# AVianEco/Softspoken

Measured on AMD Instinct MI355X. Metric: audio-seconds processed/sec (whole node), 16 kHz mono, higher is better.
Workload: dtype f16x2

## Files before the change

### softspoken_amd/csrc/conv1s.hip

```cpp
#include "kernels.h"
#include "stream16.h"
#include <algorithm>
#include <type_traits>

namespace ss {

static constexpr int kFPitch = 36;
static constexpr int kFPatch = (kMaxRows + 5) * kFPitch;

__device__ __forceinline__ float s1_from_left(float v) {
    return __builtin_bit_cast(float, __builtin_amdgcn_update_dpp(0, __builtin_bit_cast(int, v), 0x138, 0xf, 0xf, true));
}
__device__ __forceinline__ float s1_from_right(float v) {
    return __builtin_bit_cast(float, __builtin_amdgcn_update_dpp(0, __builtin_bit_cast(int, v), 0x130, 0xf, 0xf, true));
}

struct S1Row { u32x4 f[2][2]; };

template <bool TRACK>
__global__ __launch_bounds__(64 * kS1Waves) __attribute__((amdgpu_waves_per_eu(2, 2)))
void conv1_stream_kernel(ConvArgs a, int rows_per_unit, int total_units) {
    extern __shared__ __attribute__((aligned(16))) char smem[];
    char* sW = smem;
    char* sK = smem + 2 * kBank;
    char* sPrev = sK + 3 * 1024;
    float* sF = (float*)(sPrev + kS1Waves * 4096);

    const int tid = threadIdx.x, lane = tid & 63, wave = __builtin_amdgcn_readfirstlane(tid >> 6);
    const int hh = lane >> 5, m = lane & 31;
    for (int p = tid; p < 2 * kBank / 16; p += 64 * kS1Waves) *(u32x4*)(sW + p * 16) = *(const u32x4*)((const char*)a.wpk + (size_t)p * 16);
    u32x4 wf_hi, wf_lo, wr;
    {
        const float* w9 = a.first_w;
        auto wv = [&](int t) { return w9[t * 32 + m]; };
        auto hi2 = [&](float x, float y) { return pack_f16(x, y); };
        auto lo2 = [&](float x, float y) { return split_lo(pack_f16(x, y), x, y); };
        auto lo1 = [&](float x) { return x - (float)(_Float16)x; };
        const float b1 = a.first_b[m], b2 = a.bias[m], r1 = a.rank1_w[m];
        if (hh == 0) {
            wf_hi = u32x4{hi2(wv(0), wv(1)), hi2(wv(2), b1), hi2(wv(3), wv(4)), hi2(wv(5), lo1(b1))};
            wf_lo = u32x4{lo2(wv(0), wv(1)), lo2(wv(2), 0.f) & 0xffffu, lo2(wv(3), wv(4)), lo2(wv(5), 0.f) & 0xffffu};
            wr = u32x4{hi2(r1, r1), hi2(lo1(r1), b2), hi2(lo1(b2), 0.f), 0u};
        } else {
            wf_hi = u32x4{hi2(wv(6), wv(7)), hi2(wv(8), 0.f), 0u, 0u};
            wf_lo = u32x4{lo2(wv(6), wv(7)), lo2(wv(8), 0.f), 0u, 0u};
            wr = u32x4{0u, 0u, 0u, 0u};
        }
    }
    if (tid < 64) { *(u32x4*)(sK + 1024 + lane * 16) = wf_lo; *(u32x4*)(sK + 2048 + lane * 16) = wr; }
    const uint32_t kOneHi = 0x3c000000u;
    const char* sKl = sK + lane * 16;
    __syncthreads();

    const char* wl_base = sW + lane * 16;
#ifdef SS_DEVBUILD
    uint32_t st_sum[7] = {0u, 0u, 0u, 0u, 0u, 0u, 0u}, st_prev = 0;
    auto stamp = [&](int seg) {
        if (a.stamps) { const uint32_t t = (uint32_t)__builtin_amdgcn_s_memtime(); if (seg >= 0) st_sum[seg] += t - st_prev; st_prev = t; }
    };
#else
    auto stamp = [&](int) {};
#endif
    uint32_t ovf = 0;

    for (int unit = (int)blockIdx.x * kS1Waves + wave; unit < total_units; unit += (int)gridDim.x * kS1Waves) {
        stamp(-1);
        const int bands = kH / rows_per_unit;
        const int s = unit % kStrips, b = (unit / kStrips) % bands, n = unit / (kStrips * bands);
        const int x0 = kStripCols * s - 1, y0 = b * rows_per_unit;
        const int x = x0 + m;
        const bool col_in = (unsigned)x < (unsigned)kW;
        const uint32_t keep = col_in ? 0xffffffffu : 0u;
        const bool edge_strip = s == 0 || s == kStrips - 1;
        const bool st_lane = m >= 1 && m <= kStripCols && x < kW;
        const bool pl_lane = st_lane && (m & 1) && m < kStripCols;
        float* pf = sF + wave * kFPatch;
        {
            const float* fn = a.rank1_src + (size_t)n * kH * kW;
            const int nrow = rows_per_unit + 4;
            const int c = lane < 34 ? lane : 33, gx = x0 - 1 + c;
            const bool cok = lane < 34 && (unsigned)gx < (unsigned)kW;
            const int gxc = min(max(gx, 0), kW - 1);
            asm volatile("s_waitcnt lgkmcnt(0)" ::: "memory");
            bool fbad = false;
            constexpr int NR = kMaxRows + 4;
            float tv[NR];
#pragma unroll
            for (int j = 0; j < NR; ++j) {
                const int gy = y0 - 2 + j;
                const bool ok = cok && (unsigned)gy < (unsigned)kH && j < nrow;
                const float t = fn[(size_t)min(max(gy, 0), kH - 1) * kW + gxc];
                fbad |= (__builtin_bit_cast(uint32_t, t) & 0x7f800000u) == 0x7f800000u;
                tv[j] = ok ? t : 0.f;
            }
#pragma unroll
            for (int j = 0; j < NR; ++j)
                if (lane < 34 && j < nrow) pf[j * kFPitch + c] = tv[j];
            if (fbad) ovf = 0x7c007c00u;
        }
        const float* pl = pf + m;

        S1Row H0, H1, H2;
        char* prevp = sPrev + wave * 4096 + lane * 16;
#pragma unroll
        for (int q = 0; q < 2; ++q)
#pragma unroll
            for (int pl = 0; pl < 2; ++pl) { H0.f[q][pl] = u32x4{0u, 0u, 0u, 0u}; H1.f[q][pl] = u32x4{0u, 0u, 0u, 0u}; H2.f[q][pl] = u32x4{0u, 0u, 0u, 0u}; }

        f32x4 fa = {0.f, 0.f, 0.f, 0.f}, fb = fa;
        float fcen = 0.f;
        auto request = [&](int r) {
            const float* q0 = pl + (r - y0 + 1 + 2 * hh) * kFPitch;
            fa = f32x4{q0[0], q0[1], q0[2], 0.f};
            const float* q1 = q0 + (hh ? 0 : kFPitch);
            fb = f32x4{q1[0], q1[1], q1[2], 0.f};
            fcen = pl[(r - y0 + 1) * kFPitch + 1];
        };
        auto produce = [&](int r, S1Row& Hn, const u32x4& kwl) {
            if ((unsigned)r < (unsigned)kH) {
                const f32x4 oa = fa;
                const f32x4 ob = hh ? f32x4{0.f, 0.f, 0.f, 0.f} : fb;
                uint32_t bh[4], bl[4];
                bh[0] = pack_f16(oa[0], oa[1]); bl[0] = split_lo(bh[0], oa[0], oa[1]);
                bh[1] = pack_f16(oa[2], 0.f);   bl[1] = split_lo(bh[1], oa[2], 0.f);
                bh[2] = pack_f16(ob[0], ob[1]); bl[2] = split_lo(bh[2], ob[0], ob[1]);
                bh[3] = pack_f16(ob[2], 0.f);   bl[3] = split_lo(bh[3], ob[2], 0.f);
                if (!hh) { bh[1] |= kOneHi; bh[3] |= kOneHi; }
                const u32x4 boph = {bh[0], bh[1], bh[2], bh[3]}, bopl = {bl[0], bl[1], bl[2], bl[3]};
                f32x16 h;
#pragma unroll
                for (int i = 0; i < 16; ++i) h[i] = 0.f;
                h = mfma16<true>(wf_hi, bopl, h);
                h = mfma16<true>(kwl, boph, h);
                h = mfma16<true>(wf_hi, boph, h);
#pragma unroll
                for (int g = 0; g < 4; ++g)
#pragma unroll
                    for (int hq = 0; hq < 2; ++hq) {
                        const float v0 = relu_i(h[4 * g + 2 * hq]), v1 = relu_i(h[4 * g + 2 * hq + 1]);
                        const uint32_t ph = pack_f16(v0, v1);
                        if constexpr (TRACK) ovf = pk_max_u16(ovf, ph);
                        Hn.f[g >> 1][0][2 * (g & 1) + hq] = ph;
                        Hn.f[g >> 1][1][2 * (g & 1) + hq] = split_lo(ph, v0, v1);
                    }
                if (edge_strip) {
#pragma unroll
                    for (int q = 0; q < 2; ++q)
#pragma unroll
                        for (int pl = 0; pl < 2; ++pl)
#pragma unroll
                            for (int e = 0; e < 4; ++e) Hn.f[q][pl][e] &= keep;
                }
            } else {
#pragma unroll
                for (int q = 0; q < 2; ++q)
#pragma unroll
                    for (int pl = 0; pl < 2; ++pl) Hn.f[q][pl] = u32x4{0u, 0u, 0u, 0u};
            }
        };

        auto row_step = [&](int y, const S1Row& Ha, const S1Row& Hb, S1Row& Hn) {
            const float fc = fcen;
            stamp(-1);
            constexpr int PD = 2, RS = PD + 1;
            u32x4 wh[RS], wl[RS];
            auto rd = [&](int g) {
                const int dy = g / 6, q = (g / 3) & 1, dx = g % 3;
                const int off = ((dy * 3 + dx) * 2 + q) * 1024;
                wh[g % RS] = *(const u32x4*)(wl_base + off);
                wl[g % RS] = *(const u32x4*)(wl_base + kBank + off);
            };
            const u32x4 wrq = *(const u32x4*)(sKl + 2048), kwl = *(const u32x4*)(sKl + 1024);
#pragma unroll
            for (int g = 0; g < PD; ++g) rd(g);
            __builtin_amdgcn_sched_barrier(0);
            produce(y + 1, Hn, kwl);
            request(y + 2);
            stamp(1);
            f32x16 pm, p0, pp;
#pragma unroll
            for (int i = 0; i < 16; ++i) { pm[i] = 0.f; p0[i] = 0.f; pp[i] = 0.f; }
            {
                const uint32_t fh = pack_f16(fc, fc);
                const uint32_t fl = split_lo(fh, fc, fc);
                u32x4 bop = {(fh & 0xffffu) | (fl << 16), (fh & 0xffffu) | kOneHi, 0x3c00u, 0u};
                if (hh) bop = u32x4{0u, 0u, 0u, 0u};
                p0 = mfma16<true>(wrq, bop, p0);
            }
            __builtin_amdgcn_sched_barrier(0);
            stamp(4);
            {
#ifdef SS_DEVBUILD
                if (!(a.relu & 32))
#endif
#pragma unroll
                for (int g = 0; g < 18; ++g) {
                    const int dy = g / 6, q = (g / 3) & 1, dx = g % 3;
                    const S1Row& Hr = dy == 0 ? Ha : (dy == 1 ? Hb : Hn);
                    const u32x4 xh = Hr.f[q][0], xl = Hr.f[q][1];
                    if (g + PD < 18) rd(g + PD);
                    __builtin_amdgcn_sched_barrier(0);
                    f32x16& acc = dx == 0 ? pm : (dx == 1 ? p0 : pp);
                    acc = mfma16<true>(wh[g % RS], xl, acc);
                    acc = mfma16<true>(wl[g % RS], xh, acc);
                    acc = mfma16<true>(wh[g % RS], xh, acc);
                    __builtin_amdgcn_sched_barrier(0);
                }
            }
            __builtin_amdgcn_sched_barrier(0);
            stamp(0);
            float v[16];
#pragma unroll
            for (int i = 0; i < 16; ++i) {
                float t = p0[i] + s1_from_left(pm[i]);
                t = t + s1_from_right(pp[i]);
                v[i] = relu_i(t);
            }
            auto store_rows = [&](const float (&val)[16], char* dst, bool on, auto track_c) {
                constexpr bool track = TRACK && decltype(track_c)::value;
                uint32_t kh[8], kl[8];
#pragma unroll
                for (int i = 0; i < 8; ++i) {
                    kh[i] = pack_f16(val[2 * i], val[2 * i + 1]);
                    if (track) ovf = pk_max_u16(ovf, kh[i]);
                    kl[i] = split_lo(kh[i], val[2 * i], val[2 * i + 1]);
                }
                half_swap(kh[0], kh[2]); half_swap(kh[1], kh[3]); half_swap(kh[4], kh[6]); half_swap(kh[5], kh[7]);
                half_swap(kl[0], kl[2]); half_swap(kl[1], kl[3]); half_swap(kl[4], kl[6]); half_swap(kl[5], kl[7]);
#ifdef SS_DEVBUILD
                if (a.relu & 16) on = false;
#endif
                if (on) {
                    *(u32x4*)(dst) = u32x4{kh[0], kh[1], kh[2], kh[3]};
                    *(u32x4*)(dst + 32) = u32x4{kh[4], kh[5], kh[6], kh[7]};
                    *(u32x4*)(dst + a.lo_delta) = u32x4{kl[0], kl[1], kl[2], kl[3]};
                    *(u32x4*)(dst + a.lo_delta + 32) = u32x4{kl[4], kl[5], kl[6], kl[7]};
                }
            };
            f32x4 prv[4];
            if (y & 1) {
#pragma unroll
                for (int g = 0; g < 4; ++g) prv[g] = *(const f32x4*)(prevp + g * 1024);
            }
            __builtin_amdgcn_sched_barrier(0);
            store_rows(v, (char*)a.out + (((size_t)n * kH + y) * kW + (size_t)max(x, 0)) * (kC * 2) + hh * 16, st_lane, std::true_type{});
            stamp(2);
#ifdef SS_DEVBUILD
            if (a.relu & 64) return;
#endif
            if (y & 1) {
                float pv[16], prev[16];
#pragma unroll
                for (int g = 0; g < 4; ++g) {
                    prev[4 * g] = prv[g][0]; prev[4 * g + 1] = prv[g][1]; prev[4 * g + 2] = prv[g][2]; prev[4 * g + 3] = prv[g][3];
                }
#pragma unroll
                for (int i = 0; i < 16; ++i) {
                    const int t = max(__builtin_bit_cast(int, prev[i]), __builtin_bit_cast(int, v[i]));
                    pv[i] = __builtin_bit_cast(float, max(t, __builtin_amdgcn_update_dpp(0, t, 0x130, 0xf, 0xf, true)));
                }
                store_rows(pv, (char*)a.pool_out + (((size_t)n * (kH / 2) + (y >> 1)) * (kW / 2) + (size_t)(max(x, 0) >> 1)) * (kC * 2) + hh * 16, pl_lane,
                           std::false_type{});
            } else {
#pragma unroll
                for (int g = 0; g < 4; ++g) *(f32x4*)(prevp + g * 1024) = f32x4{v[4 * g], v[4 * g + 1], v[4 * g + 2], v[4 * g + 3]};
            }
            stamp(3);
#ifdef SS_DEVBUILD
            ++st_sum[5];
#endif
        };
        request(y0 - 1); produce(y0 - 1, H0, *(const u32x4*)(sKl + 1024));
        request(y0);     produce(y0, H1, *(const u32x4*)(sKl + 1024));
        request(y0 + 1);
        stamp(6);
        int k = 0;
        for (; k + 3 <= rows_per_unit; k += 3) {
            row_step(y0 + k, H0, H1, H2);
            row_step(y0 + k + 1, H1, H2, H0);
            row_step(y0 + k + 2, H2, H0, H1);
        }
        if (k < rows_per_unit) {
            row_step(y0 + k, H0, H1, H2);
            if (k + 1 < rows_per_unit) row_step(y0 + k + 1, H1, H2, H0);
        }
    }
#ifdef SS_DEVBUILD
    if (a.stamps && lane == 0) {
        uint32_t* p = (uint32_t*)a.stamps + ((size_t)blockIdx.x * kS1Waves + wave) * 16;
        for (int i = 0; i < 7; ++i) p[i] = st_sum[i];
    }
#endif
    if (((ovf & 0x7fff7fffu) + 0x04000400u) & 0x80008000u) atomicOr(a.range_flag, 1);
}

static constexpr int kFPatch16 = (kMaxRows + 6) * kFPitch;

template <bool TRACK>
__global__ __launch_bounds__(64 * kS1Waves) __attribute__((amdgpu_waves_per_eu(2, 2)))
void conv1_stream16_kernel(ConvArgs a, int rows_per_unit, int total_units) {
    extern __shared__ __attribute__((aligned(16))) char smem[];
    char* sW = smem;
    char* sK = smem + 2 * kBank;
    char* sPrev = sK + 4 * 1024;
    float* sF = (float*)(sPrev + kS1Waves * 2048);

    const int tid = threadIdx.x, lane = tid & 63, wave = __builtin_amdgcn_readfirstlane(tid >> 6);
    const int g = lane >> 4, c = lane & 15;
    for (int p = tid; p < 2 * kBank / 16; p += 64 * kS1Waves) *(u32x4*)(sW + p * 16) = *(const u32x4*)((const char*)a.wpk + (size_t)p * 16);
    u32x4 wf1[2];
    {
        const float* w9 = a.first_w;
        auto hi2 = [&](float x, float y) { return pack_f16(x, y); };
        auto lo2 = [&](float x, float y) { return split_lo(pack_f16(x, y), x, y); };
        auto lo1 = [&](float x) { return x - (float)(_Float16)x; };
#pragma unroll
        for (int u = 0; u < 2; ++u) {
            const int ch = 8 * (c >> 2) + 4 * u + (c & 3);
            auto wv = [&](int t) { return w9[t * 32 + ch]; };
            const float b1 = a.first_b[ch], b2 = a.bias[ch], r1 = a.rank1_w[ch];
            u32x4 lo = {0u, 0u, 0u, 0u}, wr = {0u, 0u, 0u, 0u};
            if ((g & 1) == 0) {
                wf1[u] = u32x4{hi2(wv(0), wv(1)), hi2(wv(2), 0.f), hi2(wv(3), wv(4)), hi2(wv(5), 0.f)};
                if (g == 0) lo = u32x4{lo2(wv(0), wv(1)), lo2(wv(2), 0.f) & 0xffffu, lo2(wv(3), wv(4)), lo2(wv(5), 0.f) & 0xffffu};
            } else {
                wf1[u] = g == 1 ? u32x4{hi2(wv(6), wv(7)), hi2(wv(8), b1), hi2(lo1(b1), 0.f), 0u} : u32x4{hi2(wv(6), wv(7)), hi2(wv(8), 0.f), 0u, 0u};
                if (g == 1) lo = u32x4{lo2(wv(6), wv(7)), lo2(wv(8), 0.f) & 0xffffu, 0u, 0u};
            }
            if (g == 0) wr = u32x4{hi2(r1, r1), hi2(lo1(r1), b2), hi2(lo1(b2), 0.f), 0u};
            if (tid < 64) { *(u32x4*)(sK + u * 1024 + lane * 16) = lo; *(u32x4*)(sK + (2 + u) * 1024 + lane * 16) = wr; }
        }
    }
    if (lane < kFPitch) sF[wave * kFPatch16 + (kMaxRows + 5) * kFPitch + lane] = 0.f;
    const uint32_t one1 = g == 1 ? 0x3c000000u : 0u, one2 = g == 1 ? 0x00003c00u : 0u;
    const bool lo_group = g >= 2;
    const char* sKl = sK + lane * 16;
    __syncthreads();

    const char* wl_base = sW + lane * 16;
#ifdef SS_DEVBUILD
    uint32_t st_sum[7] = {0u, 0u, 0u, 0u, 0u, 0u, 0u}, st_prev = 0;
    auto stamp = [&](int seg) {
        if (a.stamps) { const uint32_t t = (uint32_t)__builtin_amdgcn_s_memtime(); if (seg >= 0) st_sum[seg] += t - st_prev; st_prev = t; }
    };
#else
    auto stamp = [&](int) {};
#endif
    uint32_t ovf = 0;

    for (int unit = (int)blockIdx.x * kS1Waves + wave; unit < total_units; unit += (int)gridDim.x * kS1Waves) {
        stamp(-1);
        const int bands = kH / rows_per_unit;
        const int s = unit % kStrips, b = (unit / kStrips) % bands, n = unit / (kStrips * bands);
        const int x0 = kStripCols * s - 1, y0 = b * rows_per_unit;
        const bool edge_strip = s == 0 || s == kStrips - 1;
        uint32_t keep[2]; bool st_lane[2];
        int xt[2];
#pragma unroll
        for (int t = 0; t < 2; ++t) {
            const int mm = 2 * c + t;
            xt[t] = x0 + mm;
            keep[t] = (unsigned)xt[t] < (unsigned)kW ? 0xffffffffu : 0u;
            st_lane[t] = mm >= 1 && mm <= kStripCols && xt[t] < kW;
        }
        const bool pl_lane = st_lane[1] && 2 * c + 1 < kStripCols;
        float* pf = sF + wave * kFPatch16;
        {
            const float* fn = a.rank1_src + (size_t)n * kH * kW;
            const int nrow = rows_per_unit + 4;
            const int cc = lane < 34 ? lane : 33, gx = x0 - 1 + cc;
            const bool cok = lane < 34 && (unsigned)gx < (unsigned)kW;
            const int gxc = min(max(gx, 0), kW - 1);
            asm volatile("s_waitcnt lgkmcnt(0)" ::: "memory");
            bool fbad = false;
            constexpr int NR = kMaxRows + 4;
            float tv[NR];
#pragma unroll
            for (int j = 0; j < NR; ++j) {
                const int gy = y0 - 2 + j;
                const bool ok = cok && (unsigned)gy < (unsigned)kH && j < nrow;
                const float t = fn[(size_t)min(max(gy, 0), kH - 1) * kW + gxc];
                fbad |= (__builtin_bit_cast(uint32_t, t) & 0x7f800000u) == 0x7f800000u;
                tv[j] = ok ? t : 0.f;
            }
#pragma unroll
            for (int j = 0; j < NR; ++j)
                if (lane < 34 && j < nrow) pf[j * kFPitch + cc] = tv[j];
            if (fbad) ovf = 0x7c007c00u;
        }
        const float* pcol = pf + 2 * c;
        const float* zrow = pf + (kMaxRows + 5) * kFPitch + 2 * c;

        S16Row H0, H1, H2;
        char* prevp = sPrev + wave * 2048 + lane * 16;
        float fa[2][3], fb[2][3], fcen[2];
        auto request = [&](int r) {
            const float* q0 = pcol + (r - y0 + 1 + 2 * (g & 1)) * kFPitch;
            const float* q1 = (g & 1) ? zrow : q0 + kFPitch;
#pragma unroll
            for (int t = 0; t < 2; ++t) {
                fa[t][0] = q0[t]; fa[t][1] = q0[t + 1]; fa[t][2] = q0[t + 2];
                fb[t][0] = q1[t]; fb[t][1] = q1[t + 1]; fb[t][2] = q1[t + 2];
                fcen[t] = pcol[(r - y0 + 1) * kFPitch + t + 1];
            }
        };
        auto zero_row = [&](S16Row& Hn) {
#pragma unroll
            for (int t = 0; t < 2; ++t)
#pragma unroll
                for (int pl = 0; pl < 2; ++pl) Hn.f[t][pl] = u32x4{0u, 0u, 0u, 0u};
        };
        auto produce = [&](int r, S16Row& Hn, const u32x4 (&kwl)[2]) {
            if ((unsigned)r < (unsigned)kH) {
#pragma unroll
                for (int t = 0; t < 2; ++t) {
                    uint32_t bh[4], bl[4];
                    bh[0] = pack_f16(fa[t][0], fa[t][1]); bl[0] = split_lo(bh[0], fa[t][0], fa[t][1]);
                    bh[1] = pack_f16(fa[t][2], 0.f);      bl[1] = split_lo(bh[1], fa[t][2], 0.f);
                    bh[2] = pack_f16(fb[t][0], fb[t][1]); bl[2] = split_lo(bh[2], fb[t][0], fb[t][1]);
                    bh[3] = pack_f16(fb[t][2], 0.f);      bl[3] = split_lo(bh[3], fb[t][2], 0.f);
                    bh[1] |= one1; bh[2] |= one2;
                    const u32x4 bop = lo_group ? u32x4{bl[0], bl[1], bl[2], bl[3]} : u32x4{bh[0], bh[1], bh[2], bh[3]};
                    uint32_t ph[2][2], pl[2][2];
#pragma unroll
                    for (int u = 0; u < 2; ++u) {
                        f32x4 h = {0.f, 0.f, 0.f, 0.f};
                        h = s16_mfma(kwl[u], bop, h);
                        h = s16_mfma(wf1[u], bop, h);
#pragma unroll
                        for (int hq = 0; hq < 2; ++hq) {
                            const float v0 = relu_i(h[2 * hq]), v1 = relu_i(h[2 * hq + 1]);
                            ph[u][hq] = pack_f16(v0, v1);
                            if constexpr (TRACK) ovf = pk_max_u16(ovf, ph[u][hq]);
                            pl[u][hq] = split_lo(ph[u][hq], v0, v1);
                        }
                    }
                    Hn.f[t][0] = u32x4{ph[0][0], ph[0][1], ph[1][0], ph[1][1]};
                    Hn.f[t][1] = u32x4{pl[0][0], pl[0][1], pl[1][0], pl[1][1]};
                    if (edge_strip) {
#pragma unroll
                        for (int pq = 0; pq < 2; ++pq)
#pragma unroll
                            for (int e = 0; e < 4; ++e) Hn.f[t][pq][e] &= keep[t];
                    }
                }
            } else zero_row(Hn);
        };

        auto row_step = [&](int y, const S16Row& Ha, const S16Row& Hb, S16Row& Hn) {
            const float fc[2] = {fcen[0], fcen[1]};
            stamp(-1);
            S16Ring ring;
            const u32x4 kwl[2] = {*(const u32x4*)(sKl), *(const u32x4*)(sKl + 1024)};
            const u32x4 wrq[2] = {*(const u32x4*)(sKl + 2048), *(const u32x4*)(sKl + 3072)};
            ring.rd(wl_base, 0);
            __builtin_amdgcn_sched_barrier(0);
            produce(y + 1, Hn, kwl);
            request(y + 2);
            stamp(1);
            f32x4 P[3][2][2];
#pragma unroll
            for (int t = 0; t < 2; ++t) {
                const uint32_t fh = pack_f16(fc[t], fc[t]);
                const uint32_t fl = split_lo(fh, fc[t], fc[t]);
                u32x4 bop = {(fh & 0xffffu) | (fl << 16), (fh & 0xffffu) | 0x3c000000u, 0x3c00u, 0u};
                if (g != 0) bop = u32x4{0u, 0u, 0u, 0u};
#pragma unroll
                for (int u = 0; u < 2; ++u) {
                    P[0][t][u] = f32x4{0.f, 0.f, 0.f, 0.f}; P[2][t][u] = f32x4{0.f, 0.f, 0.f, 0.f};
                    P[1][t][u] = s16_mfma(wrq[u], bop, f32x4{0.f, 0.f, 0.f, 0.f});
                }
            }
            __builtin_amdgcn_sched_barrier(0);
            stamp(4);
            s16_taps(ring, wl_base, Ha, Hb, Hn, P, [](int) {});
            stamp(0);
            float v[2][2][4];
            s16_combine(P, v);
            auto store_px = [&](const float (&val)[2][4], char* dst, bool on, auto track_c) {
                constexpr bool track = TRACK && decltype(track_c)::value;
                uint32_t kh[4], kl[4];
                s16_split_px(val, kh, kl);
                if (track) {
#pragma unroll
                    for (int i = 0; i < 4; ++i) ovf = pk_max_u16(ovf, kh[i]);
                }
                if (on) {
                    *(u32x4*)(dst) = u32x4{kh[0], kh[1], kh[2], kh[3]};
                    *(u32x4*)(dst + a.lo_delta) = u32x4{kl[0], kl[1], kl[2], kl[3]};
                }
            };
            f32x4 prv[2];
            if (y & 1) { prv[0] = *(const f32x4*)(prevp); prv[1] = *(const f32x4*)(prevp + 1024); }
            __builtin_amdgcn_sched_barrier(0);
#pragma unroll
            for (int t = 0; t < 2; ++t)
                store_px(v[t], (char*)a.out + (((size_t)n * kH + y) * kW + (size_t)max(xt[t], 0)) * (kC * 2) + g * 16, st_lane[t], std::true_type{});
            stamp(2);
            float cm[2][4];
#pragma unroll
            for (int u = 0; u < 2; ++u)
#pragma unroll
                for (int r = 0; r < 4; ++r)
                    cm[u][r] = __int_as_float(max(__float_as_int(v[1][u][r]), s16_shl1(__float_as_int(v[0][u][r]))));
            if (y & 1) {
#pragma unroll
                for (int u = 0; u < 2; ++u)
#pragma unroll
                    for (int r = 0; r < 4; ++r) cm[u][r] = __int_as_float(max(__float_as_int(cm[u][r]), __float_as_int(prv[u][r])));
                store_px(cm, (char*)a.pool_out + (((size_t)n * (kH / 2) + (y >> 1)) * (kW / 2) + (size_t)(max(xt[1], 0) >> 1)) * (kC * 2) + g * 16, pl_lane,
                         std::false_type{});
            } else {
                *(f32x4*)(prevp) = f32x4{cm[0][0], cm[0][1], cm[0][2], cm[0][3]};
                *(f32x4*)(prevp + 1024) = f32x4{cm[1][0], cm[1][1], cm[1][2], cm[1][3]};
            }
            stamp(3);
#ifdef SS_DEVBUILD
            ++st_sum[5];
#endif
        };
        {
            const u32x4 kwl0[2] = {*(const u32x4*)(sKl), *(const u32x4*)(sKl + 1024)};
            request(y0 - 1); produce(y0 - 1, H0, kwl0);
            request(y0);     produce(y0, H1, kwl0);
            request(y0 + 1);
        }
        stamp(6);
        int k = 0;
        for (; k + 3 <= rows_per_unit; k += 3) {
            row_step(y0 + k, H0, H1, H2);
            row_step(y0 + k + 1, H1, H2, H0);
            row_step(y0 + k + 2, H2, H0, H1);
        }
        if (k < rows_per_unit) {
            row_step(y0 + k, H0, H1, H2);
            if (k + 1 < rows_per_unit) row_step(y0 + k + 1, H1, H2, H0);
        }
    }
#ifdef SS_DEVBUILD
    if (a.stamps && lane == 0) {
        uint32_t* p = (uint32_t*)a.stamps + ((size_t)blockIdx.x * kS1Waves + wave) * 16;
        for (int i = 0; i < 7; ++i) p[i] = st_sum[i];
    }
#endif
    if (((ovf & 0x7fff7fffu) + 0x04000400u) & 0x80008000u) atomicOr(a.range_flag, 1);
}

bool conv1_stream_supports(const ConvArgs& a) {
    return a.H == kH && a.W == kW && a.Cout == kC && a.first_w && a.first_b && a.rank1_src && a.rank1_w && a.wpk && a.out && a.pool_out &&
           a.lo_delta != 0 && a.range_flag && a.N > 0;
}
const char* conv1_stream_variant(const ConvArgs& a, int form) {
    if (form == 16) return a.plain ? "conv1_stream16_kernel<false>" : "conv1_stream16_kernel<true>";
    return a.plain ? "conv1_stream_kernel<false>" : "conv1_stream_kernel<true>";
}
size_t conv1_stream_weight_bytes() { return 2 * (size_t)kBank; }

hipError_t launch_conv1_stream(const ConvArgs& a, int form, int rows_per_unit, int num_cus, hipStream_t s) {
    if (!conv1_stream_supports(a) || rows_per_unit < 2 || (rows_per_unit & 1) || kH % rows_per_unit || rows_per_unit > kMaxRows) return hipErrorInvalidValue;
    const int64_t total = (int64_t)a.N * (kH / rows_per_unit) * kStrips;
    if (total >= (int64_t)1 << 30) return hipErrorInvalidValue;
    const int cus = num_cus > 0 ? num_cus : 256;
    const int grid = (int)std::min<int64_t>(cus, (total + kS1Waves - 1) / kS1Waves);
    static std::atomic<uint64_t> attr_done{0}, attr_done2{0}, attr_done3{0}, attr_done4{0};
    if (form == 16) {
        const size_t lds = 2 * (size_t)kBank + 4 * 1024 + (size_t)kS1Waves * 2048 + (size_t)kS1Waves * kFPatch16 * sizeof(float);
        if (hipError_t e = allow_full_lds((const void*)conv1_stream16_kernel<true>, attr_done3)) return e;
        if (hipError_t e = allow_full_lds((const void*)conv1_stream16_kernel<false>, attr_done4)) return e;
        if (a.plain) hipLaunchKernelGGL(conv1_stream16_kernel<false>, dim3(grid), dim3(64 * kS1Waves), lds, s, a, rows_per_unit, (int)total);
        else hipLaunchKernelGGL(conv1_stream16_kernel<true>, dim3(grid), dim3(64 * kS1Waves), lds, s, a, rows_per_unit, (int)total);
        return hipGetLastError();
    }
#ifdef SS_DEVBUILD
    const size_t lds = 2 * (size_t)kBank + 3 * 1024 + (size_t)kS1Waves * 4096 + (size_t)kS1Waves * kFPatch * sizeof(float);
    if (hipError_t e = allow_full_lds((const void*)conv1_stream_kernel<true>, attr_done)) return e;
    if (hipError_t e = allow_full_lds((const void*)conv1_stream_kernel<false>, attr_done2)) return e;
    if (a.plain) hipLaunchKernelGGL(conv1_stream_kernel<false>, dim3(grid), dim3(64 * kS1Waves), lds, s, a, rows_per_unit, (int)total);
    else hipLaunchKernelGGL(conv1_stream_kernel<true>, dim3(grid), dim3(64 * kS1Waves), lds, s, a, rows_per_unit, (int)total);
    return hipGetLastError();
#else
    (void)attr_done; (void)attr_done2;
    return hipErrorInvalidValue;
#endif
}

}
```

### softspoken_amd/csrc/stream16.h

```cpp
#pragma once
#include "mfma_util.h"

namespace ss {

static constexpr int kH = 128, kW = 256, kC = 32;
static constexpr int kStrips = 9, kStripCols = 30;
static constexpr int kBank = 9 * 2 * 1024;
static constexpr int kS1Waves = 8;
static constexpr int kMaxRows = 32;

struct S16Row { u32x4 f[2][2]; };

__device__ __forceinline__ f32x4 s16_mfma(const u32x4& a, const u32x4& b, const f32x4& c) {
    return __builtin_amdgcn_mfma_f32_16x16x32_f16(__builtin_bit_cast(f16x8, a), __builtin_bit_cast(f16x8, b), c, 0, 0, 0);
}
__device__ __forceinline__ int s16_shr1(int v) { return __builtin_amdgcn_update_dpp(0, v, 0x111, 0xf, 0xf, true); }
__device__ __forceinline__ int s16_shl1(int v) { return __builtin_amdgcn_update_dpp(0, v, 0x101, 0xf, 0xf, true); }
__device__ __forceinline__ float s16_shr1f(float v) { return __int_as_float(s16_shr1(__float_as_int(v))); }
__device__ __forceinline__ float s16_shl1f(float v) { return __int_as_float(s16_shl1(__float_as_int(v))); }

struct S16Ring {
    u32x4 wh[2][2], wl[2][2];
    __device__ __forceinline__ void rd(const char* wl_base, int tap) {
#pragma unroll
        for (int u = 0; u < 2; ++u) {
            wh[tap & 1][u] = *(const u32x4*)(wl_base + (tap * 2 + u) * 1024);
            wl[tap & 1][u] = *(const u32x4*)(wl_base + kBank + (tap * 2 + u) * 1024);
        }
    }
};

template <typename AfterTap>
__device__ __forceinline__ void s16_taps(S16Ring& ring, const char* wl_base, const S16Row& Ha, const S16Row& Hb, const S16Row& Hn, f32x4 (&P)[3][2][2],
                                         AfterTap&& after_tap) {
#pragma unroll
    for (int tap = 0; tap < 9; ++tap) {
        const int dy = tap / 3, dx = tap % 3;
        const S16Row& Hr = dy == 0 ? Ha : (dy == 1 ? Hb : Hn);
        if (tap + 1 < 9) ring.rd(wl_base, tap + 1);
        __builtin_amdgcn_sched_barrier(0);
#pragma unroll
        for (int pr = 0; pr < 3; ++pr)
#pragma unroll
            for (int u = 0; u < 2; ++u)
#pragma unroll
                for (int t = 0; t < 2; ++t)
                    P[dx][t][u] = s16_mfma(pr == 1 ? ring.wl[tap & 1][u] : ring.wh[tap & 1][u], Hr.f[t][pr == 0 ? 1 : 0], P[dx][t][u]);
        __builtin_amdgcn_sched_barrier(0);
        if (tap + 1 < 9) after_tap(tap);
    }
    __builtin_amdgcn_sched_barrier(0);
}

__device__ __forceinline__ void s16_combine(const f32x4 (&P)[3][2][2], float (&v)[2][2][4]) {
#pragma unroll
    for (int u = 0; u < 2; ++u)
#pragma unroll
        for (int r = 0; r < 4; ++r) {
            v[0][u][r] = relu_i(P[1][0][u][r] + s16_shr1f(P[0][1][u][r]) + P[2][1][u][r]);
            v[1][u][r] = relu_i(P[1][1][u][r] + P[0][0][u][r] + s16_shl1f(P[2][0][u][r]));
        }
}

static constexpr int kStrips32 = 8;

struct S16RowH { u32x4 f[2][2]; u32x4 h[2]; };

__device__ __forceinline__ u32x4 s16_shr1_halo(const u32x4& v, const u32x4& halo) {
    u32x4 r;
#pragma unroll
    for (int e = 0; e < 4; ++e) r[e] = (uint32_t)__builtin_amdgcn_update_dpp((int)halo[e], (int)v[e], 0x111, 0xf, 0xf, false);
    return r;
}
__device__ __forceinline__ u32x4 s16_shl1_halo(const u32x4& v, const u32x4& halo) {
    u32x4 r;
#pragma unroll
    for (int e = 0; e < 4; ++e) r[e] = (uint32_t)__builtin_amdgcn_update_dpp((int)halo[e], (int)v[e], 0x101, 0xf, 0xf, false);
    return r;
}

struct S16Ring3 {
    u32x4 wh[3][2], wl[3][2];
    __device__ __forceinline__ void rd(int slot, const char* hi, const char* lo, int step) {
#pragma unroll
        for (int u = 0; u < 2; ++u) { wh[slot][u] = *(const u32x4*)(hi + u * step); wl[slot][u] = *(const u32x4*)(lo + u * step); }
    }
    __device__ __forceinline__ void rd_tap(int slot, const char* wl_base, int tap) { rd(slot, wl_base + tap * 2048, wl_base + kBank + tap * 2048, 1024); }
};

__device__ __forceinline__ void s16_products(const S16Ring3& ring, int slot, const u32x4 (&B)[2], f32x4 (&Pt)[2]) {
#pragma unroll
    for (int pr = 0; pr < 3; ++pr)
#pragma unroll
        for (int u = 0; u < 2; ++u) Pt[u] = s16_mfma(pr == 1 ? ring.wl[slot][u] : ring.wh[slot][u], B[pr == 0 ? 1 : 0], Pt[u]);
}

template <typename Last, typename AfterTap>
__device__ __forceinline__ void s16_taps_shifted(S16Ring3& ring, const char* wl_base, const S16RowH& Ha, const S16RowH& Hb, const S16RowH& Hn,
                                                 f32x4 (&P)[2][2], Last&& before_last, AfterTap&& after_tap) {
#pragma unroll
    for (int tap = 0; tap < 9; ++tap) {
        const int dy = tap / 3, dx = tap % 3 - 1, slot = tap & 1;
        const S16RowH& Hr = dy == 0 ? Ha : (dy == 1 ? Hb : Hn);
        if (tap + 1 < 9) ring.rd_tap(slot ^ 1, wl_base, tap + 1); else before_last();
        u32x4 B[2][2];
#pragma unroll
        for (int pq = 0; pq < 2; ++pq) {
            B[0][pq] = dx == 0 ? Hr.f[0][pq] : (dx < 0 ? s16_shr1_halo(Hr.f[1][pq], Hr.h[pq]) : Hr.f[1][pq]);
            B[1][pq] = dx == 0 ? Hr.f[1][pq] : (dx < 0 ? Hr.f[0][pq] : s16_shl1_halo(Hr.f[0][pq], Hr.h[pq]));
        }
        __builtin_amdgcn_sched_barrier(0);
#pragma unroll
        for (int pr = 0; pr < 3; ++pr)
#pragma unroll
            for (int u = 0; u < 2; ++u)
#pragma unroll
                for (int t = 0; t < 2; ++t)
                    P[t][u] = s16_mfma(pr == 1 ? ring.wl[slot][u] : ring.wh[slot][u], B[t][pr == 0 ? 1 : 0], P[t][u]);
        __builtin_amdgcn_sched_barrier(0);
        after_tap(tap);
    }
}

__device__ __forceinline__ void s16_split_px(const float (&val)[2][4], uint32_t (&kh)[4], uint32_t (&kl)[4]) {
#pragma unroll
    for (int i = 0; i < 4; ++i) {
        const float e0 = val[i >> 1][2 * (i & 1)], e1 = val[i >> 1][2 * (i & 1) + 1];
        kh[i] = pack_f16(e0, e1);
        kl[i] = split_lo(kh[i], e0, e1);
    }
}

}
```

Before: 33960.

## Restructure stream16 conv1 into 32-column strips with precomputed shifted halo operands

Changes the fp16 stream conv1 kernel from 9 overlapping 30-column strips to 8 non-overlapping 32-column strips. Each lane now computes its halo columns, and the left- and right-shifted operands are prebuilt per row, so the three partial accumulators and the DPP combine step are gone. The f32 patch in shared memory is stored already split into hi/lo f16 words and assembled with byte-perm, and the edge masking and store predicates are removed. The cost is an extra halo produce pass (a third MFMA set per row), larger row state in registers, and more LDS. The correctness of the removed boundary masks relies on the halo selection.

After: 34390, median of 6. 1.3% higher.

```diff
diff --git a/softspoken_amd/csrc/conv1s.hip b/softspoken_amd/csrc/conv1s.hip
--- a/softspoken_amd/csrc/conv1s.hip
+++ b/softspoken_amd/csrc/conv1s.hip
@@ -294,7 +294,13 @@
     if (((ovf & 0x7fff7fffu) + 0x04000400u) & 0x80008000u) atomicOr(a.range_flag, 1);
 }
 
-static constexpr int kFPatch16 = (kMaxRows + 6) * kFPitch;
+static constexpr int kFPatch16 = (kMaxRows + 7) * kFPitch;
+
+__device__ __forceinline__ uint32_t s1_split_word(float x) {
+    uint32_t w = pack_f16(x, 0.f);
+    asm("v_fma_mixhi_f16 %0, %0, -1.0, %1 op_sel_hi:[1,0,0]" : "+v"(w) : "v"(x));
+    return w;
+}
 
 template <bool TRACK>
 __global__ __launch_bounds__(64 * kS1Waves) __attribute__((amdgpu_waves_per_eu(2, 2)))
@@ -303,7 +309,7 @@
     char* sW = smem;
     char* sK = smem + 2 * kBank;
     char* sPrev = sK + 4 * 1024;
-    float* sF = (float*)(sPrev + kS1Waves * 2048);
+    uint32_t* sF = (uint32_t*)(sPrev + kS1Waves * 2048);
 
     const int tid = threadIdx.x, lane = tid & 63, wave = __builtin_amdgcn_readfirstlane(tid >> 6);
     const int g = lane >> 4, c = lane & 15;
@@ -331,9 +337,9 @@
             if (tid < 64) { *(u32x4*)(sK + u * 1024 + lane * 16) = lo; *(u32x4*)(sK + (2 + u) * 1024 + lane * 16) = wr; }
         }
     }
-    if (lane < kFPitch) sF[wave * kFPatch16 + (kMaxRows + 5) * kFPitch + lane] = 0.f;
-    const uint32_t one1 = g == 1 ? 0x3c000000u : 0u, one2 = g == 1 ? 0x00003c00u : 0u;
-    const bool lo_group = g >= 2;
+    if (lane < kFPitch) { sF[wave * kFPatch16 + (kMaxRows + 5) * kFPitch + lane] = 0u; sF[wave * kFPatch16 + (kMaxRows + 6) * kFPitch + lane] = 0x3c00u; }
+    const uint32_t selg = g >= 2 ? 0x07060302u : 0x05040100u;
+    const uint32_t one1 = g == 1 ? 0x00003c00u : 0u;
     const char* sKl = sK + lane * 16;
     __syncthreads();
 
@@ -351,25 +357,16 @@
     for (int unit = (int)blockIdx.x * kS1Waves + wave; unit < total_units; unit += (int)gridDim.x * kS1Waves) {
         stamp(-1);
         const int bands = kH / rows_per_unit;
-        const int s = unit % kStrips, b = (unit / kStrips) % bands, n = unit / (kStrips * bands);
-        const int x0 = kStripCols * s - 1, y0 = b * rows_per_unit;
-        const bool edge_strip = s == 0 || s == kStrips - 1;
-        uint32_t keep[2]; bool st_lane[2];
-        int xt[2];
-#pragma unroll
-        for (int t = 0; t < 2; ++t) {
-            const int mm = 2 * c + t;
-            xt[t] = x0 + mm;
-            keep[t] = (unsigned)xt[t] < (unsigned)kW ? 0xffffffffu : 0u;
-            st_lane[t] = mm >= 1 && mm <= kStripCols && xt[t] < kW;
-        }
-        const bool pl_lane = st_lane[1] && 2 * c + 1 < kStripCols;
-        float* pf = sF + wave * kFPatch16;
+        const int s = unit % kStrips32, b = (unit / kStrips32) % bands, n = unit / (kStrips32 * bands);
+        const int x0 = 32 * s, y0 = b * rows_per_unit;
+        const int xc = x0 + 2 * c;
+        const uint32_t hkeep = (c < 8 ? s > 0 : s < kStrips32 - 1) ? 0xffffffffu : 0u;
+        uint32_t* pf = sF + wave * kFPatch16;
         {
             const float* fn = a.rank1_src + (size_t)n * kH * kW;
             const int nrow = rows_per_unit + 4;
-            const int cc = lane < 34 ? lane : 33, gx = x0 - 1 + cc;
-            const bool cok = lane < 34 && (unsigned)gx < (unsigned)kW;
+            const int cc = lane < kFPitch ? lane : kFPitch - 1, gx = x0 - 2 + cc;
+            const bool cok = lane < kFPitch && (unsigned)gx < (unsigned)kW;
             const int gxc = min(max(gx, 0), kW - 1);
             asm volatile("s_waitcnt lgkmcnt(0)" ::: "memory");
             bool fbad = false;
@@ -385,42 +382,50 @@
             }
 #pragma unroll
             for (int j = 0; j < NR; ++j)
-                if (lane < 34 && j < nrow) pf[j * kFPitch + cc] = tv[j];
+                if (lane < kFPitch && j < nrow) pf[j * kFPitch + cc] = s1_split_word(tv[j]);
             if (fbad) ovf = 0x7c007c00u;
         }
-        const float* pcol = pf + 2 * c;
-        const float* zrow = pf + (kMaxRows + 5) * kFPitch + 2 * c;
-
-        S16Row H0, H1, H2;
+        const uint32_t* pcol = pf + 2 * c + 1;
+        const uint32_t* hcol = pf + (c < 8 ? 0 : 33);
+        const int zoff = (kMaxRows + (g == 1 ? 6 : 5)) * kFPitch;
+        const uint32_t selh = hkeep ? selg : 0x0c0c0c0cu;
+
+        S16RowS H0, H1, H2;
         char* prevp = sPrev + wave * 2048 + lane * 16;
-        float fa[2][3], fb[2][3], fcen[2];
+        char* orow = (char*)a.out + (((size_t)n * kH + y0) * kW + (size_t)xc) * (kC * 2) + g * 16;
+        char* prow = (char*)a.pool_out + (((size_t)n * (kH / 2) + (y0 >> 1)) * (kW / 2) + (size_t)(xc >> 1)) * (kC * 2) + g * 16;
+        uint32_t fa[3][3], fb[3][3], fcen[2];
+        u32x4 kwl[2], wrq[2];
+        auto request_k = [&] {
+            kwl[0] = *(const u32x4*)(sKl); kwl[1] = *(const u32x4*)(sKl + 1024);
+            wrq[0] = *(const u32x4*)(sKl + 2048); wrq[1] = *(const u32x4*)(sKl + 3072);
+        };
         auto request = [&](int r) {
-            const float* q0 = pcol + (r - y0 + 1 + 2 * (g & 1)) * kFPitch;
-            const float* q1 = (g & 1) ? zrow : q0 + kFPitch;
-#pragma unroll
-            for (int t = 0; t < 2; ++t) {
-                fa[t][0] = q0[t]; fa[t][1] = q0[t + 1]; fa[t][2] = q0[t + 2];
-                fb[t][0] = q1[t]; fb[t][1] = q1[t + 1]; fb[t][2] = q1[t + 2];
-                fcen[t] = pcol[(r - y0 + 1) * kFPitch + t + 1];
-            }
-        };
-        auto zero_row = [&](S16Row& Hn) {
-#pragma unroll
-            for (int t = 0; t < 2; ++t)
-#pragma unroll
-                for (int pl = 0; pl < 2; ++pl) Hn.f[t][pl] = u32x4{0u, 0u, 0u, 0u};
-        };
-        auto produce = [&](int r, S16Row& Hn, const u32x4 (&kwl)[2]) {
+            const int ro = (r - y0 + 1 + 2 * (g & 1)) * kFPitch, ro1 = (g & 1) ? zoff : ro + kFPitch;
+#pragma unroll
+            for (int t = 0; t < 3; ++t) {
+                const uint32_t* q = t < 2 ? pcol + t : hcol;
+#pragma unroll
+                for (int i = 0; i < 3; ++i) { fa[t][i] = q[ro + i]; fb[t][i] = q[ro1 + i]; }
+            }
+#pragma unroll
+            for (int t = 0; t < 2; ++t) fcen[t] = pcol[(r - y0 + 1) * kFPitch + t + 1];
+        };
+        auto zero_row = [&](S16RowS& Hn) {
+#pragma unroll
+            for (int pq = 0; pq < 2; ++pq) {
+                Hn.f[0][pq] = u32x4{0u, 0u, 0u, 0u}; Hn.f[1][pq] = u32x4{0u, 0u, 0u, 0u};
+                Hn.l[pq] = u32x4{0u, 0u, 0u, 0u}; Hn.r[pq] = u32x4{0u, 0u, 0u, 0u};
+            }
+        };
+        auto produce = [&](int r, S16RowS& Hn) {
             if ((unsigned)r < (unsigned)kH) {
-#pragma unroll
-                for (int t = 0; t < 2; ++t) {
-                    uint32_t bh[4], bl[4];
-                    bh[0] = pack_f16(fa[t][0], fa[t][1]); bl[0] = split_lo(bh[0], fa[t][0], fa[t][1]);
-                    bh[1] = pack_f16(fa[t][2], 0.f);      bl[1] = split_lo(bh[1], fa[t][2], 0.f);
-                    bh[2] = pack_f16(fb[t][0], fb[t][1]); bl[2] = split_lo(bh[2], fb[t][0], fb[t][1]);
-                    bh[3] = pack_f16(fb[t][2], 0.f);      bl[3] = split_lo(bh[3], fb[t][2], 0.f);
-                    bh[1] |= one1; bh[2] |= one2;
-                    const u32x4 bop = lo_group ? u32x4{bl[0], bl[1], bl[2], bl[3]} : u32x4{bh[0], bh[1], bh[2], bh[3]};
+                u32x4 halo[2];
+#pragma unroll
+                for (int t = 0; t < 3; ++t) {
+                    const uint32_t sel = t == 2 ? selh : selg;
+                    const u32x4 bop = {__builtin_amdgcn_perm(fa[t][1], fa[t][0], sel), __builtin_amdgcn_perm(one1, fa[t][2], sel),
+                                       __builtin_amdgcn_perm(fb[t][1], fb[t][0], sel), __builtin_amdgcn_perm(0u, fb[t][2], sel)};
                     uint32_t ph[2][2], pl[2][2];
 #pragma unroll
                     for (int u = 0; u < 2; ++u) {
@@ -431,53 +436,47 @@
                         for (int hq = 0; hq < 2; ++hq) {
                             const float v0 = relu_i(h[2 * hq]), v1 = relu_i(h[2 * hq + 1]);
                             ph[u][hq] = pack_f16(v0, v1);
-                            if constexpr (TRACK) ovf = pk_max_u16(ovf, ph[u][hq]);
+                            if constexpr (TRACK) { if (t < 2) ovf = pk_max_u16(ovf, ph[u][hq]); }
                             pl[u][hq] = split_lo(ph[u][hq], v0, v1);
                         }
                     }
-                    Hn.f[t][0] = u32x4{ph[0][0], ph[0][1], ph[1][0], ph[1][1]};
-                    Hn.f[t][1] = u32x4{pl[0][0], pl[0][1], pl[1][0], pl[1][1]};
-                    if (edge_strip) {
-#pragma unroll
-                        for (int pq = 0; pq < 2; ++pq)
-#pragma unroll
-                            for (int e = 0; e < 4; ++e) Hn.f[t][pq][e] &= keep[t];
-                    }
-                }
+                    const u32x4 xh = {ph[0][0], ph[0][1], ph[1][0], ph[1][1]}, xl = {pl[0][0], pl[0][1], pl[1][0], pl[1][1]};
+                    if (t < 2) { Hn.f[t][0] = xh; Hn.f[t][1] = xl; } else { halo[0] = xh; halo[1] = xl; }
+                }
+                s16_make_shifted(Hn, halo);
             } else zero_row(Hn);
         };
 
-        auto row_step = [&](int y, const S16Row& Ha, const S16Row& Hb, S16Row& Hn) {
-            const float fc[2] = {fcen[0], fcen[1]};
+        auto row_step = [&](int y, const S16RowS& Ha, const S16RowS& Hb, S16RowS& Hn) {
+            const uint32_t fc[2] = {fcen[0], fcen[1]};
             stamp(-1);
-            S16Ring ring;
-            const u32x4 kwl[2] = {*(const u32x4*)(sKl), *(const u32x4*)(sKl + 1024)};
-            const u32x4 wrq[2] = {*(const u32x4*)(sKl + 2048), *(const u32x4*)(sKl + 3072)};
-            ring.rd(wl_base, 0);
-            __builtin_amdgcn_sched_barrier(0);
-            produce(y + 1, Hn, kwl);
+            S16Ring3 ring;
+            ring.rd_tap(0, wl_base, 0);
+            __builtin_amdgcn_sched_barrier(0);
+            produce(y + 1, Hn);
             request(y + 2);
             stamp(1);
-            f32x4 P[3][2][2];
+            f32x4 P[2][2];
 #pragma unroll
             for (int t = 0; t < 2; ++t) {
-                const uint32_t fh = pack_f16(fc[t], fc[t]);
-                const uint32_t fl = split_lo(fh, fc[t], fc[t]);
-                u32x4 bop = {(fh & 0xffffu) | (fl << 16), (fh & 0xffffu) | 0x3c000000u, 0x3c00u, 0u};
-                if (g != 0) bop = u32x4{0u, 0u, 0u, 0u};
-#pragma unroll
-                for (int u = 0; u < 2; ++u) {
-                    P[0][t][u] = f32x4{0.f, 0.f, 0.f, 0.f}; P[2][t][u] = f32x4{0.f, 0.f, 0.f, 0.f};
-                    P[1][t][u] = s16_mfma(wrq[u], bop, f32x4{0.f, 0.f, 0.f, 0.f});
-                }
+                const u32x4 bop = {fc[t], __builtin_amdgcn_perm(0x3c003c00u, fc[t], 0x05040100u), 0x3c00u, 0u};
+#pragma unroll
+                for (int u = 0; u < 2; ++u) P[t][u] = s16_mfma(wrq[u], bop, f32x4{0.f, 0.f, 0.f, 0.f});
             }
             __builtin_amdgcn_sched_barrier(0);
             stamp(4);
-            s16_taps(ring, wl_base, Ha, Hb, Hn, P, [](int) {});
+            s16_taps_shifted(ring, wl_base, Ha, Hb, Hn, P, [] {}, [](int) {});
+            __builtin_amdgcn_sched_barrier(0);
             stamp(0);
+            request_k();
             float v[2][2][4];
-            s16_combine(P, v);
-            auto store_px = [&](const float (&val)[2][4], char* dst, bool on, auto track_c) {
+#pragma unroll
+            for (int t = 0; t < 2; ++t)
+#pragma unroll
+                for (int u = 0; u < 2; ++u)
+#pragma unroll
+                    for (int r = 0; r < 4; ++r) v[t][u][r] = relu_i(P[t][u][r]);
+            auto store_px = [&](const float (&val)[2][4], char* dst, auto track_c) {
                 constexpr bool track = TRACK && decltype(track_c)::value;
                 uint32_t kh[4], kl[4];
                 s16_split_px(val, kh, kl);
@@ -485,31 +484,27 @@
 #pragma unroll
                     for (int i = 0; i < 4; ++i) ovf = pk_max_u16(ovf, kh[i]);
                 }
-                if (on) {
-                    *(u32x4*)(dst) = u32x4{kh[0], kh[1], kh[2], kh[3]};
-                    *(u32x4*)(dst + a.lo_delta) = u32x4{kl[0], kl[1], kl[2], kl[3]};
-                }
+                *(u32x4*)(dst) = u32x4{kh[0], kh[1], kh[2], kh[3]};
+                *(u32x4*)(dst + a.lo_delta) = u32x4{kl[0], kl[1], kl[2], kl[3]};
             };
             f32x4 prv[2];
             if (y & 1) { prv[0] = *(const f32x4*)(prevp); prv[1] = *(const f32x4*)(prevp + 1024); }
             __builtin_amdgcn_sched_barrier(0);
-#pragma unroll
-            for (int t = 0; t < 2; ++t)
-                store_px(v[t], (char*)a.out + (((size_t)n * kH + y) * kW + (size_t)max(xt[t], 0)) * (kC * 2) + g * 16, st_lane[t], std::true_type{});
+            char* o = orow + (size_t)(y - y0) * (kW * kC * 2);
+#pragma unroll
+            for (int t = 0; t < 2; ++t) store_px(v[t], o + t * (kC * 2), std::true_type{});
             stamp(2);
             float cm[2][4];
 #pragma unroll
             for (int u = 0; u < 2; ++u)
 #pragma unroll
-                for (int r = 0; r < 4; ++r)
-                    cm[u][r] = __int_as_float(max(__float_as_int(v[1][u][r]), s16_shl1(__float_as_int(v[0][u][r]))));
+                for (int r = 0; r < 4; ++r) cm[u][r] = __int_as_float(max(__float_as_int(v[0][u][r]), __float_as_int(v[1][u][r])));
             if (y & 1) {
 #pragma unroll
                 for (int u = 0; u < 2; ++u)
 #pragma unroll
                     for (int r = 0; r < 4; ++r) cm[u][r] = __int_as_float(max(__float_as_int(cm[u][r]), __float_as_int(prv[u][r])));
-                store_px(cm, (char*)a.pool_out + (((size_t)n * (kH / 2) + (y >> 1)) * (kW / 2) + (size_t)(max(xt[1], 0) >> 1)) * (kC * 2) + g * 16, pl_lane,
-                         std::false_type{});
+                store_px(cm, prow + (size_t)((y - y0) >> 1) * ((kW / 2) * kC * 2), std::false_type{});
             } else {
                 *(f32x4*)(prevp) = f32x4{cm[0][0], cm[0][1], cm[0][2], cm[0][3]};
                 *(f32x4*)(prevp + 1024) = f32x4{cm[1][0], cm[1][1], cm[1][2], cm[1][3]};
@@ -519,12 +514,10 @@
             ++st_sum[5];
 #endif
         };
-        {
-            const u32x4 kwl0[2] = {*(const u32x4*)(sKl), *(const u32x4*)(sKl + 1024)};
-            request(y0 - 1); produce(y0 - 1, H0, kwl0);
-            request(y0);     produce(y0, H1, kwl0);
-            request(y0 + 1);
-        }
+        request_k();
+        request(y0 - 1); produce(y0 - 1, H0);
+        request(y0);     produce(y0, H1);
+        request(y0 + 1);
         stamp(6);
         int k = 0;
         for (; k + 3 <= rows_per_unit; k += 3) {
@@ -558,7 +551,7 @@
 
 hipError_t launch_conv1_stream(const ConvArgs& a, int form, int rows_per_unit, int num_cus, hipStream_t s) {
     if (!conv1_stream_supports(a) || rows_per_unit < 2 || (rows_per_unit & 1) || kH % rows_per_unit || rows_per_unit > kMaxRows) return hipErrorInvalidValue;
-    const int64_t total = (int64_t)a.N * (kH / rows_per_unit) * kStrips;
+    const int64_t total = (int64_t)a.N * (kH / rows_per_unit) * (form == 16 ? kStrips32 : kStrips);
     if (total >= (int64_t)1 << 30) return hipErrorInvalidValue;
     const int cus = num_cus > 0 ? num_cus : 256;
     const int grid = (int)std::min<int64_t>(cus, (total + kS1Waves - 1) / kS1Waves);
diff --git a/softspoken_amd/csrc/stream16.h b/softspoken_amd/csrc/stream16.h
--- a/softspoken_amd/csrc/stream16.h
+++ b/softspoken_amd/csrc/stream16.h
@@ -5,66 +5,18 @@
 
 static constexpr int kH = 128, kW = 256, kC = 32;
 static constexpr int kStrips = 9, kStripCols = 30;
+static constexpr int kStrips32 = 8;
 static constexpr int kBank = 9 * 2 * 1024;
 static constexpr int kS1Waves = 8;
 static constexpr int kMaxRows = 32;
 
 struct S16Row { u32x4 f[2][2]; };
+struct S16RowH { u32x4 f[2][2]; u32x4 h[2]; };
+struct S16RowS { u32x4 f[2][2]; u32x4 l[2], r[2]; };
 
 __device__ __forceinline__ f32x4 s16_mfma(const u32x4& a, const u32x4& b, const f32x4& c) {
     return __builtin_amdgcn_mfma_f32_16x16x32_f16(__builtin_bit_cast(f16x8, a), __builtin_bit_cast(f16x8, b), c, 0, 0, 0);
 }
-__device__ __forceinline__ int s16_shr1(int v) { return __builtin_amdgcn_update_dpp(0, v, 0x111, 0xf, 0xf, true); }
-__device__ __forceinline__ int s16_shl1(int v) { return __builtin_amdgcn_update_dpp(0, v, 0x101, 0xf, 0xf, true); }
-__device__ __forceinline__ float s16_shr1f(float v) { return __int_as_float(s16_shr1(__float_as_int(v))); }
-__device__ __forceinline__ float s16_shl1f(float v) { return __int_as_float(s16_shl1(__float_as_int(v))); }
-
-struct S16Ring {
-    u32x4 wh[2][2], wl[2][2];
-    __device__ __forceinline__ void rd(const char* wl_base, int tap) {
-#pragma unroll
-        for (int u = 0; u < 2; ++u) {
-            wh[tap & 1][u] = *(const u32x4*)(wl_base + (tap * 2 + u) * 1024);
-            wl[tap & 1][u] = *(const u32x4*)(wl_base + kBank + (tap * 2 + u) * 1024);
-        }
-    }
-};
-
-template <typename AfterTap>
-__device__ __forceinline__ void s16_taps(S16Ring& ring, const char* wl_base, const S16Row& Ha, const S16Row& Hb, const S16Row& Hn, f32x4 (&P)[3][2][2],
-                                         AfterTap&& after_tap) {
-#pragma unroll
-    for (int tap = 0; tap < 9; ++tap) {
-        const int dy = tap / 3, dx = tap % 3;
-        const S16Row& Hr = dy == 0 ? Ha : (dy == 1 ? Hb : Hn);
-        if (tap + 1 < 9) ring.rd(wl_base, tap + 1);
-        __builtin_amdgcn_sched_barrier(0);
-#pragma unroll
-        for (int pr = 0; pr < 3; ++pr)
-#pragma unroll
-            for (int u = 0; u < 2; ++u)
-#pragma unroll
-                for (int t = 0; t < 2; ++t)
-                    P[dx][t][u] = s16_mfma(pr == 1 ? ring.wl[tap & 1][u] : ring.wh[tap & 1][u], Hr.f[t][pr == 0 ? 1 : 0], P[dx][t][u]);
-        __builtin_amdgcn_sched_barrier(0);
-        if (tap + 1 < 9) after_tap(tap);
-    }
-    __builtin_amdgcn_sched_barrier(0);
-}
-
-__device__ __forceinline__ void s16_combine(const f32x4 (&P)[3][2][2], float (&v)[2][2][4]) {
-#pragma unroll
-    for (int u = 0; u < 2; ++u)
-#pragma unroll
-        for (int r = 0; r < 4; ++r) {
-            v[0][u][r] = relu_i(P[1][0][u][r] + s16_shr1f(P[0][1][u][r]) + P[2][1][u][r]);
-            v[1][u][r] = relu_i(P[1][1][u][r] + P[0][0][u][r] + s16_shl1f(P[2][0][u][r]));
-        }
-}
-
-static constexpr int kStrips32 = 8;
-
-struct S16RowH { u32x4 f[2][2]; u32x4 h[2]; };
 
 __device__ __forceinline__ u32x4 s16_shr1_halo(const u32x4& v, const u32x4& halo) {
     u32x4 r;
@@ -77,6 +29,20 @@
 #pragma unroll
     for (int e = 0; e < 4; ++e) r[e] = (uint32_t)__builtin_amdgcn_update_dpp((int)halo[e], (int)v[e], 0x101, 0xf, 0xf, false);
     return r;
+}
+__device__ __forceinline__ u32x4 s16_operand(const S16RowH& H, int dx, int t, int pq) {
+    if (dx == 0) return H.f[t][pq];
+    if (dx < 0) return t == 0 ? s16_shr1_halo(H.f[1][pq], H.h[pq]) : H.f[0][pq];
+    return t == 0 ? H.f[1][pq] : s16_shl1_halo(H.f[0][pq], H.h[pq]);
+}
+__device__ __forceinline__ u32x4 s16_operand(const S16RowS& H, int dx, int t, int pq) {
+    if (dx == 0) return H.f[t][pq];
+    if (dx < 0) return t == 0 ? H.l[pq] : H.f[0][pq];
+    return t == 0 ? H.f[1][pq] : H.r[pq];
+}
+__device__ __forceinline__ void s16_make_shifted(S16RowS& H, const u32x4 (&halo)[2]) {
+#pragma unroll
+    for (int pq = 0; pq < 2; ++pq) { H.l[pq] = s16_shr1_halo(H.f[1][pq], halo[pq]); H.r[pq] = s16_shl1_halo(H.f[0][pq], halo[pq]); }
 }
 
 struct S16Ring3 {
@@ -95,20 +61,17 @@
         for (int u = 0; u < 2; ++u) Pt[u] = s16_mfma(pr == 1 ? ring.wl[slot][u] : ring.wh[slot][u], B[pr == 0 ? 1 : 0], Pt[u]);
 }
 
-template <typename Last, typename AfterTap>
-__device__ __forceinline__ void s16_taps_shifted(S16Ring3& ring, const char* wl_base, const S16RowH& Ha, const S16RowH& Hb, const S16RowH& Hn,
+template <typename Row, typename Last, typename AfterTap>
+__device__ __forceinline__ void s16_taps_shifted(S16Ring3& ring, const char* wl_base, const Row& Ha, const Row& Hb, const Row& Hn,
                                                  f32x4 (&P)[2][2], Last&& before_last, AfterTap&& after_tap) {
 #pragma unroll
     for (int tap = 0; tap < 9; ++tap) {
         const int dy = tap / 3, dx = tap % 3 - 1, slot = tap & 1;
-        const S16RowH& Hr = dy == 0 ? Ha : (dy == 1 ? Hb : Hn);
+        const Row& Hr = dy == 0 ? Ha : (dy == 1 ? Hb : Hn);
         if (tap + 1 < 9) ring.rd_tap(slot ^ 1, wl_base, tap + 1); else before_last();
         u32x4 B[2][2];
 #pragma unroll
-        for (int pq = 0; pq < 2; ++pq) {
-            B[0][pq] = dx == 0 ? Hr.f[0][pq] : (dx < 0 ? s16_shr1_halo(Hr.f[1][pq], Hr.h[pq]) : Hr.f[1][pq]);
-            B[1][pq] = dx == 0 ? Hr.f[1][pq] : (dx < 0 ? Hr.f[0][pq] : s16_shl1_halo(Hr.f[0][pq], Hr.h[pq]));
-        }
+        for (int pq = 0; pq < 2; ++pq) { B[0][pq] = s16_operand(Hr, dx, 0, pq); B[1][pq] = s16_operand(Hr, dx, 1, pq); }
         __builtin_amdgcn_sched_barrier(0);
 #pragma unroll
         for (int pr = 0; pr < 3; ++pr)
```
